# G1OJS/PyFT8

Hardware: AMD Instinct MI355X
Metric: FT8 15-s frames decoded/sec (higher is better)
Workload: dtype f32

## Files before the change

pyft8_amd/csrc/kernels/cycle_spectrum.hpp:

```cpp
#ifndef FT8RX_CYCLE_SPECTRUM_HPP
#define FT8RX_CYCLE_SPECTRUM_HPP

FT8_DEV void cyc_a_load(const int16_t* __restrict__ a, int n2b, int tid, uint32_t (&raw)[10]) {
#pragma unroll
    for (int q = 0; q < 10; q++) {
        const int i = tid + 256 * q, ic = i < 2400 ? i : 0;
        const int c = ic & 7, n1 = ic >> 3;
        const int m = 320 * n1 + n2b + c;
        const int inb = (2 * m < FT8RX_NSAMP) ? -1 : 0;
        raw[q] = *reinterpret_cast<const uint32_t*>(a + ((2 * m) & inb)) & (uint32_t)inb;
    }
}
FT8_DEV void cyc_a_frame(const uint32_t (&raw)[10], cpx* bufA, cpx* bufB, cpx* __restrict__ out, const Tables& T, int n2b, int tid) {
#pragma unroll
    for (int q = 0; q < 10; q++) {
        const int i = tid + 256 * q;
        if (i < 2400) bufA[(i & 7) * 300 + (i >> 3)] = make_float2((float)(int16_t)(raw[q] & 0xFFFFu), (float)(int16_t)(raw[q] >> 16));
    }
    cpx w[10];
#pragma unroll
    for (int q = 0; q < 10; q++) { const int i = tid + 256 * q, ic = i < 2400 ? i : 0; w[q] = T.W96000[(n2b + (ic & 7)) * (ic >> 3)]; }
    __syncthreads();
    cpx* r = lds_fft<300, 5, 5, 4, 3>(bufA, bufB, T.W300, 8, tid, 256);
#pragma unroll
    for (int q = 0; q < 10; q++) {
        const int i = tid + 256 * q;
        if (i < 2400) { const int c = i & 7, k1 = i >> 3; out[k1 * 320 + n2b + c] = cmul(r[c * 300 + k1], w[q]); }
    }
}
__global__ __launch_bounds__(256) void k_cyc_a(const int16_t* __restrict__ audio, cpx* __restrict__ A, Tables T) {
    __shared__ cpx bufA[8 * 300];
    __shared__ cpx bufB[8 * 300];
    static_assert(320 / 8 == 8 * 5, "the tile map below assumes 40 column tiles = 8 XCDs x 5");
    const int tile = (blockIdx.x & 7) * 5 + (blockIdx.x >> 3);
    const int f = blockIdx.y, tid = threadIdx.x, n2b = 8 * tile;
    uint32_t raw[10];
    cyc_a_load(audio + (size_t)f * FT8RX_NSAMP, n2b, tid, raw);
    cyc_a_frame(raw, bufA, bufB, A + (size_t)f * 96000, T, n2b, tid);
}

#define CYC_BC_BLOCKS 39
#define CYC_BC_GRID 40
FT8_DEV int cyc_bc_row(int b, int r) {
    if (b == CYC_BC_BLOCKS - 1) return (r == 0) ? 0 : 150;
    const int k1a = 1 + 4 * b;
    return (r < 4) ? k1a + r : 300 - (k1a + (r - 4));
}
FT8_DEV void cyc_bc_load(const cpx* __restrict__ in, int b, int tid, cpx (&v)[10]) {
#pragma unroll
    for (int q = 0; q < 10; q++) {
        const int i = tid + 256 * q, r = i / 320, c = i - 320 * r;
        v[q] = in[(size_t)cyc_bc_row(b, r) * 320 + c];
    }
}
FT8_DEV void cyc_bc_frame(const cpx (&v)[10], cpx* bufA, cpx* bufB, cpx* __restrict__ out, const Tables& T, int b, int tid) {
#pragma unroll
    for (int q = 0; q < 10; q++) bufA[tid + 256 * q] = v[q];
    __syncthreads();
    cpx* z = lds_fft<320, 8, 8, 5>(bufA, bufB, T.W320, 8, tid, 256);
    const bool special = (b == CYC_BC_BLOCKS - 1);
    constexpr int NK2 = (FT8RX_SPEC_BINS + 299) / 300;
    static_assert(NK2 <= 320, "k2 range of the 320-point row transforms");
    for (int i = tid; i < 8 * NK2; i += 256) {
        const int half = i / (4 * NK2), j = i - half * (4 * NK2), rr = j & 3, k2 = j >> 2;
        const int r = 4 * half + rr;
        int pr, pk2;
        if (special) {
            if (r >= 2) continue;
            pr = r;
            pk2 = (r == 0) ? ((320 - k2) % 320) : 319 - k2;
        } else {
            pr = (r < 4) ? r + 4 : r - 4;
            pk2 = 319 - k2;
        }
        const int k = cyc_bc_row(b, r) + 300 * k2;
        if (k >= FT8RX_SPEC_BINS) continue;
        const cpx p = z[r * 320 + k2], q = z[pr * 320 + pk2];
        const float er = 0.5f * (p.x + q.x), ei = 0.5f * (p.y - q.y);
        const float orr = 0.5f * (p.y + q.y), oi = 0.5f * (q.x - p.x);
        const cpx w = T.WR192k[k];
        out[k] = make_float2(er + (w.x * orr - w.y * oi), ei + (w.x * oi + w.y * orr));
    }
}
__global__ __launch_bounds__(256) void k_cyc_bc(const cpx* __restrict__ A, cpx* __restrict__ spec, Tables T) {
    __shared__ cpx bufA[8 * 320];
    __shared__ cpx bufB[8 * 320];
    static_assert(CYC_BC_GRID == 8 * 5 && CYC_BC_BLOCKS <= CYC_BC_GRID, "tile map: 40 slots = 8 XCDs x 5");
    const int f = blockIdx.y, tid = threadIdx.x, b = (blockIdx.x & 7) * 5 + (blockIdx.x >> 3);
    if (b >= CYC_BC_BLOCKS) return;
    cpx v[10];
    cyc_bc_load(A + (size_t)f * 96000, b, tid, v);
    cyc_bc_frame(v, bufA, bufB, spec + (size_t)f * FT8RX_SPEC_BINS, T, b, tid);
}

#endif
```

pyft8_amd/csrc/kernels/fine_sync.hpp:

```cpp
#ifndef FT8RX_FINE_SYNC_HPP
#define FT8RX_FINE_SYNC_HPP

#ifndef FINE_NT
#define FINE_NT 128
#endif
#ifndef FINE_WV
#define FINE_WV 3
#endif
#define FINE_INV 0.0003125f

#ifdef FINE_TIMING
__device__ unsigned long long g_fine_t[32];
#define FT_DECL __shared__ unsigned long long ft_l[32]; if (tid < 32) ft_l[tid] = 0; __syncthreads(); unsigned long long ft_prev = __builtin_readcyclecounter();
#define FT_ARG , unsigned long long& ft_prev, unsigned long long* ft_l
#define FT_PASS , ft_prev, ft_l
#define FT(i) do { if (tid == 0) { unsigned long long ft_now = __builtin_readcyclecounter(); ft_l[i] += ft_now - ft_prev; ft_prev = __builtin_readcyclecounter(); } } while (0)
#define FT_FLUSH do { __syncthreads(); if (tid < 32) atomicAdd(&g_fine_t[tid], ft_l[tid]); } while (0)
#else
#define FT_DECL
#define FT_ARG
#define FT_PASS
#define FT(i) do { } while (0)
#define FT_FLUSH do { } while (0)
#endif
// ... 2 lines not shown
FT8_DEV cpx fine_taper(cpx v, double t) { return make_float2((float)((double)v.x * t), (float)((double)v.y * t)); }
FT8_DEV cpx fine_conj(cpx v) { return make_float2(v.x, -v.y); }

FT8_DEV void dft8_in012(cpx* a) {
    const float h = 0.70710678f;
    const cpx a0 = a[0], a1 = a[1], a2 = a[2];
    const cpx e0 = cadd(a0, a2), e2 = csub(a0, a2);
    const cpx e1 = make_float2(a0.x + a2.y, a0.y - a2.x), e3 = make_float2(a0.x - a2.y, a0.y + a2.x);
    const cpx o1 = make_float2(h * (a1.x + a1.y), h * (a1.y - a1.x));
    const cpx o2 = make_float2(a1.y, -a1.x);
    const cpx o3 = make_float2(o1.y, -o1.x);
    a[0] = cadd(e0, a1); a[4] = csub(e0, a1);
    a[1] = cadd(e1, o1); a[5] = csub(e1, o1);
    a[2] = cadd(e2, o2); a[6] = csub(e2, o2);
    a[3] = cadd(e3, o3); a[7] = csub(e3, o3);
}
FT8_DEV void dft8_in017(cpx* a) {
    const float h = 0.70710678f;
    const cpx a0 = a[0], a1 = a[1], a7 = a[7];
    const cpx q0 = cadd(a1, a7), q2 = csub(a1, a7);
    const cpx q1 = make_float2(a1.x - a7.y, a1.y + a7.x), q3 = make_float2(a1.x + a7.y, a1.y - a7.x);
    const cpx o1 = make_float2(h * (q1.x + q1.y), h * (q1.y - q1.x));
    const cpx o2 = make_float2(q2.y, -q2.x);
    const cpx o3 = make_float2(h * (q3.y - q3.x), -(h * (q3.x + q3.y)));
    a[0] = cadd(a0, q0); a[4] = csub(a0, q0);
    a[1] = cadd(a0, o1); a[5] = csub(a0, o1);
    a[2] = cadd(a0, o2); a[6] = csub(a0, o2);
    a[3] = cadd(a0, o3); a[7] = csub(a0, o3);
}
static_assert(FINE_NT == 128, "fine_stage1 is written for 128 threads");
FT8_DEV void fine_stage1(const cpx* S, int fb, cpx* z, const cpx* __restrict__ W,
                         const double* __restrict__ taper, int tid FT_ARG) {
    const cpx zero = make_float2(0.0f, 0.0f);
    const cpx* s0 = S + fb + tid;
    const cpx* s7 = S + fb - 150 - 250 + tid;
    const cpx a00 = s0[0], a01 = s0[400];
    const cpx a10 = s0[128], a11 = s0[528];
    const cpx a20 = s0[256], a21 = s0[656];
    const bool r3 = tid < 16;
    const int t3 = r3 ? tid : 0;
    const cpx a30 = s0[384 + t3 - tid], a31 = s0[784 + t3 - tid];
    const bool has02 = tid < 50;
    const cpx a02r = s0[has02 ? 800 : 0];
    const double t02 = taper[has02 ? tid + 50 : 0];
    const bool has17 = tid >= 122;
    const cpx a17r = s7[has17 ? 128 : 250];
    const double t17 = taper[has17 ? tid - 122 : 0];
    const uint32_t m02 = has02 ? 0xFFFFFFFFu : 0u, m17 = has17 ? 0xFFFFFFFFu : 0u;
    const cpx a27r = s7[256];
    const bool tap21 = tid >= 94;
    const double t2 = taper[tap21 ? tid - 94 : tid + 6];
    const cpx a37r = s7[384 + t3 - tid];
    const double t31 = taper[34 + t3];
    const cpx t02v = fine_taper(a02r, t02), t17v = fine_taper(a17r, t17);
    const cpx a02 = make_float2(__uint_as_float(__float_as_uint(t02v.x) & m02), __uint_as_float(__float_as_uint(t02v.y) & m02));
    const cpx a17 = make_float2(__uint_as_float(__float_as_uint(t17v.x) & m17), __uint_as_float(__float_as_uint(t17v.y) & m17));
    const cpx sel2 = fine_taper(tap21 ? a21 : a27r, t2);
    const cpx b21 = tap21 ? sel2 : a21, a27 = tap21 ? a27r : sel2;
    const cpx b31 = fine_taper(a31, t31);
    cpx a[4][8];
#pragma unroll
    for (int i = 0; i < 4; i++)
#pragma unroll
        for (int j = 2; j < 7; j++) a[i][j] = zero;
    a[0][0] = fine_conj(a00); a[0][1] = fine_conj(a01); a[0][2] = fine_conj(a02); a[0][7] = zero;
    a[1][0] = fine_conj(a10); a[1][1] = fine_conj(a11); a[1][7] = fine_conj(a17);
    a[2][0] = fine_conj(a20); a[2][1] = fine_conj(b21); a[2][7] = fine_conj(a27);
    a[3][0] = fine_conj(a30); a[3][1] = fine_conj(b31); a[3][7] = fine_conj(a37r);
#pragma unroll
    for (int i = 0; i < 4; i++) {
        const int p = tid + 128 * i;
        const int pw = (i < 3) ? p : 384 + t3;
        cpx w[8];
#pragma unroll
        for (int j = 1; j < 8; j++) w[j] = W[j * pw];
        if (i == 0) dft8_in012(a[i]); else dft8_in017(a[i]);
#pragma unroll
        for (int j = 1; j < 8; j++) a[i][j] = cmul(a[i][j], w[j]);
        if (i < 3 || r3) {
#pragma unroll
            for (int j = 0; j < 8; j++) z[8 * p + j] = a[i][j];
        }
    }
    FT(1);
    __syncthreads();
    FT(2);
}
FT8_DEV void fine_stage2(cpx* z, const cpx* w400, int tid FT_ARG) {
    typedef Fused2<3200, 400, 8, 4, 4> F;
    constexpr int R = (F::groups + FINE_NT - 1) / FINE_NT;
    cpx a[R][4][4];
#pragma unroll
    for (int r = 0; r < R; r++) { const int g = tid + FINE_NT * r; if (g < F::groups) F::load_affine<200, 800>(z, g, a[r]); }
    FT(3);
    __syncthreads();
    FT(4);
#pragma unroll
    for (int r = 0; r < R; r++) {
        const int g = tid + FINE_NT * r;
        if (g < F::groups) {
            const int pp = g >> 3;
#pragma unroll
            for (int jp = 0; jp < 4; jp++) {
                dft<4>(a[r][jp]);
                const int pq = pp + 25 * jp;
#pragma unroll
                for (int j = 1; j < 4; j++) a[r][jp][j] = cmul(a[r][jp][j], w400[j * pq]);
            }
#pragma unroll
            for (int j = 0; j < 4; j++) {
                cpx b[4];
#pragma unroll
                for (int jp = 0; jp < 4; jp++) b[jp] = a[r][jp][j];
                dft<4>(b);
#pragma unroll
                for (int jp = 1; jp < 4; jp++) b[jp] = cmul(b[jp], w400[4 * jp * pp]);
#pragma unroll
                for (int jp = 0; jp < 4; jp++) a[r][jp][j] = b[jp];
            }
            F::store_affine<32, 8>(z, (g & 7) + 128 * (g >> 3), a[r]);
        }
    }
    FT(5);
    __syncthreads();
    FT(6);
}
FT8_DEV void fine_stage3(cpx* z, const cpx* __restrict__ W, int tid, int lo, int hi FT_ARG) {
    typedef Fused2<3200, 25, 128, 5, 5> F;
    constexpr int R = F::groups / FINE_NT;
    cpx a[R][5][5];
#pragma unroll
    for (int r = 0; r < R; r++) F::load_affine<128, 640>(z, tid + FINE_NT * r, a[r]);
    FT(7);
    __syncthreads();
    FT(8);
#pragma unroll
    for (int r = 0; r < R; r++) {
        const int q = tid + FINE_NT * r;
        F::compute_passA(0, a[r], W);
#pragma unroll
        for (int j = 0; j < 5; j++) {
            const int rr = q + 128 * j;
            const int first = rr + 640 * (lo / 640 + (rr < lo % 640 ? 1 : 0));
            if (first < hi && first < 3200) {
                cpx b[5];
#pragma unroll
                for (int jp = 0; jp < 5; jp++) b[jp] = a[r][jp][j];
                dft<5>(b);
#pragma unroll
                for (int jp = 0; jp < 5; jp++) z[rr + 640 * jp] = b[jp];
            }
        }
    }
    FT(9);
    __syncthreads();
    FT(10);
}
FT8_DEV void fine_fft(const cpx* S, int fb, cpx* z, const cpx* w400, const Tables& T, int tid, int lo, int hi FT_ARG) {
    FT(0);
    fine_stage1(S, fb, z, T.W3200, T.taper, tid FT_PASS);
    fine_stage2(z, w400, tid FT_PASS);
    fine_stage3(z, T.W3200, tid, lo, hi FT_PASS);
}

template <int NT>
FT8_DEV void fine_sym_quad(const cpx* z, int i0, int n2, const cpx* wq, float* mag) {
    if (i0 < 0) i0 = 0;
    if (i0 > 3168) i0 = 3168;
    cpx x[8];
#pragma unroll
    for (int n1 = 0; n1 < 8; n1++) { cpx v = z[i0 + 4 * n1 + n2]; x[n1] = make_float2(v.x * FINE_INV, -(v.y * FINE_INV)); }
    sym32_quad<NT>(x, n2, wq, mag);
}

#ifdef FT8RX_ILP_UNIT
#define FS_CS 0
#define FS_H 156
#define FS_MAG 1556
struct FsLane {
    float k[17];
    cpx g0[10];
    cpx g[10];
    double tap;
    cpx cs[2];
    int r, jlo;
};
FT8_DEV void fscore_fetch(FsLane& L, const Tables& T, int tid) {
    const int lane = tid & 63;
    const int ln = lane < 50 ? lane : 0;
    L.r = tid < 64 ? 50 + ln : ln;
    L.jlo = tid < 64 ? -2 : -1;
#pragma unroll
    for (int u = 0; u < 17; u++) L.k[u] = T.K32[900 + L.r + 100 * (L.jlo - 7 + u)];
#pragma unroll
    for (int q = 0; q < 10; q++) L.g0[q] = T.G1000[L.r + 100 * (L.jlo + q) + 150];
    L.tap = T.taper[tid < 64 ? ln : 50 + ln];
#pragma unroll
    for (int u = 0; u < 2; u++) { const int i = tid + FINE_NT * u; L.cs[u] = T.CS100[i < 156 ? i : 0]; }
}
FT8_DEV void fscore_phases(FsLane& L, const Tables& T, int nb0) {
    cpx w[10];
    {
        const int step = (((100 * nb0) % 3200) + 3200) % 3200;
        int idx = ((((L.r + 100 * L.jlo) * nb0) % 3200) + 3200) % 3200;
#pragma unroll
        for (int q = 0; q < 10; q++) { w[q] = T.W3200[idx]; idx += step; idx -= (idx >= 3200) ? 3200 : 0; }
    }
#pragma unroll
    for (int q = 0; q < 10; q++) L.g[q] = cmul(make_float2(w[q].x, -w[q].y), L.g0[q]);
}
FT8_DEV void fscore_prepare(FsLane& L, cpx* zi, const Tables& T, int nb0, int tid) {
    fscore_phases(L, T, nb0);
#pragma unroll
    for (int u = 0; u < 2; u++) { const int i = tid + FINE_NT * u; if (i < 156) zi[FS_CS + i] = L.cs[u]; }
    __syncthreads();
}
template <int NTONE>
FT8_DEV void fscore_p1(const cpx* S, int off, const FsLane& L, cpx* H, int tid FT_ARG) {
    cpx b[10];
#pragma unroll
    for (int q = 0; q < 10; q++) {
        cpx x = S[off + L.r + 100 * (L.jlo + q)];
        if (q == 0 || q == 9) x = fine_taper(x, L.tap);
        b[q] = cmul(x, L.g[q]);
    }
    FT(16);
    float hx[NTONE], hy[NTONE];
#pragma unroll
    for (int t = 0; t < NTONE; t++) { hx[t] = 0.0f; hy[t] = 0.0f; }
#pragma unroll
    for (int u = 0; u < 17; u++) {
#pragma unroll
        for (int t = 0; t < NTONE; t++) {
            const int q = u + t - 7;
            if (q >= 0 && q < 10) {
                hx[t] = __builtin_fmaf(b[q].x, L.k[u], hx[t]);
                hy[t] = __builtin_fmaf(b[q].y, L.k[u], hy[t]);
            }
        }
    }
    FT(17);
#pragma unroll
    for (int t = 0; t < NTONE; t++) H[t * 100 + L.r] = make_float2(hx[t], hy[t]);
}
FT8_DEV void dft10_fwd(const cpx* x, cpx* y) {
    cpx a0[5], a1[5];
#pragma unroll
    for (int n = 0; n < 5; n++) { const cpx u = x[(2 * n) % 10], v = x[(5 + 2 * n) % 10]; a0[n] = cadd(u, v); a1[n] = csub(u, v); }
    dft<5>(a0); dft<5>(a1);
#pragma unroll
    for (int k = 0; k < 5; k++) { y[(6 * k) % 10] = a0[k]; y[(5 + 6 * k) % 10] = a1[k]; }
}
FT8_DEV float row16_sum(float v) {
    v += __int_as_float(__builtin_amdgcn_update_dpp(0, __float_as_int(v), 0xB1, 0xf, 0xf, false));
    v += __int_as_float(__builtin_amdgcn_update_dpp(0, __float_as_int(v), 0x4E, 0xf, 0xf, false));
    v += __int_as_float(__builtin_amdgcn_update_dpp(0, __float_as_int(v), 0x141, 0xf, 0xf, false));
    v += __int_as_float(__builtin_amdgcn_update_dpp(0, __float_as_int(v), 0x140, 0xf, 0xf, false));
    return v;
}
FT8_DEV void fine_fscore(const cpx* S, int off, const FsLane& L, cpx* zi, int n, int tid FT_ARG) {
    cpx* H = zi + FS_H + (n & 1) * 700;
    float* mags = reinterpret_cast<float*>(zi + FS_MAG) + n * 56;
    const int lane = tid & 63;
    if (lane < 50) fscore_p1<7>(S, off, L, H, tid FT_PASS);
    FT(11);
    __syncthreads();
    FT(12);
    {
        const int c = tid & 15, t = tid >> 4;
        cpx acc[7];
#pragma unroll
        for (int s = 0; s < 7; s++) acc[s] = make_float2(0.0f, 0.0f);
        const cpx* Ht = H + (t < 7 ? t : 0) * 100;
#pragma unroll
        for (int i = 0; i < 2; i++) {
            const int p = c + 16 * i;
            if (i < 1 || c < 10) {
                const bool first = (i == 0 && c == 0), last = (i == 1 && c == 9);
                const cpx zero = make_float2(0.0f, 0.0f);
                const cpx h1 = Ht[p];
                cpx h2 = Ht[first ? 99 : 100 - p], h3 = Ht[50 - p], h4 = Ht[50 + p];
                if (first) { h2 = zero; h4 = zero; }
                if (last) { h3 = zero; h4 = zero; }
                const cpx P = make_float2(h1.x + h2.x, h1.y + h2.y), M = make_float2(h1.x - h2.x, h1.y - h2.y);
                const cpx P2 = make_float2(h3.x + h4.x, h3.y + h4.y), M2 = make_float2(h3.x - h4.x, h3.y - h4.y);
                const cpx A = make_float2(P.x + P2.x, P.y + P2.y), B = make_float2(P.x - P2.x, P.y - P2.y);
                const cpx C = make_float2(M.x - M2.x, M.y - M2.y), D = make_float2(M.x + M2.x, M.y + M2.y);
                acc[0] = cadd(acc[0], A);
#pragma unroll
                for (int s = 1; s < 7; s++) {
                    const cpx e = zi[FS_CS + (s - 1) * 26 + p];
                    const cpx X = (s & 1) ? B : A, Y = (s & 1) ? D : C;
                    acc[s].x = __builtin_fmaf(X.x, e.x, __builtin_fmaf(-Y.y, e.y, acc[s].x));
                    acc[s].y = __builtin_fmaf(X.y, e.x, __builtin_fmaf(Y.x, e.y, acc[s].y));
                }
            }
        }
        FT(19);
#pragma unroll
        for (int s = 0; s < 7; s++) { acc[s].x = row16_sum(acc[s].x); acc[s].y = row16_sum(acc[s].y); }
        {
            cpx v = acc[0];
#pragma unroll
            for (int s = 1; s < 7; s++) v = (c == s) ? acc[s] : v;
            const float re = v.x * FINE_INV, im = v.y * FINE_INV;
            mags[c < 7 ? c * 8 + t : 7] = sqrtf(re * re + im * im);
        }
    }
    FT(14);
}

FT8_DEV void fine_candidate(int tid, int bid, const cpx* __restrict__ spec, ft8rx_record* __restrict__ rec,
                            const int32_t* __restrict__ ncand, float* __restrict__ llr0, const Tables& T, const ft8rx_config& cfg,
                            const int32_t* __restrict__ trip, int32_t* __restrict__ t_out ,
                            float* __restrict__ t_sd, float* __restrict__ t_sgrid) {
    __shared__ cpx z[3200];
    __shared__ cpx w400[400];
    float* mg = reinterpret_cast<float*>(w400);
    static_assert(sizeof(cpx) * 400 >= sizeof(float) * 640, "mg overlays w400");
    __shared__ cpx w32[32];
    __shared__ float sc[16];
    __shared__ int ish[4];
    const int lane = tid & 63;
    int frame, ci = 0, f0, h0;
    if (trip) { frame = trip[3 * bid]; f0 = trip[3 * bid + 1]; h0 = trip[3 * bid + 2]; }
    else {
        frame = bid >> cand_shift(cfg); ci = bid & ((1 << cand_shift(cfg)) - 1);
        if (ci >= ncand[frame]) return;
        const ft8rx_record& r = rec[bid];
        if (r.status != FT8RX_ST_ACTIVE) return;
        f0 = r.f0_idx; h0 = r.h0_idx;
    }
    if (h0 < FT8RX_MIN_H0_FD || h0 > FT8RX_MAX_H0_FD) return;
    const cpx w32v = T.W32[tid & 31];
    const int fb0 = 50 * f0;
    {
        constexpr int NW = (400 + FINE_NT - 1) / FINE_NT;
        cpx wv[NW];
#pragma unroll
        for (int q = 0; q < NW; q++) { const int i = tid + FINE_NT * q; wv[q] = T.W3200[8 * (i < 400 ? i : 0)]; }
#pragma unroll
        for (int q = 0; q < NW; q++) { const int i = tid + FINE_NT * q; if (i < 400) w400[i] = wv[q]; }
        if (tid < 32) w32[tid] = w32v;
        __syncthreads();
    }
    const cpx* __restrict__ Sg = spec + (size_t)frame * FT8RX_SPEC_BINS + (fb0 - 182);
    FT_DECL
    cpx wq[8];
    sym32_twiddles(w32, tid & 3, wq);
    const int tb0 = 8 * h0 + (h0 < 0 ? 1 : 0);
    double* dsum = reinterpret_cast<double*>(mg);
    fine_fft(Sg, 182, z, w400, T, tid, tb0 - 8 + 32 * 36, tb0 + 6 + 32 * 43 FT_PASS);
    FsLane L;
    fscore_fetch(L, T, tid);
    const bool lowslice = tb0 >= 667;
    cpx* slice = z + (lowslice ? 0 : 2048);
    cpx* zi = z + (lowslice ? 1152 : 0);
    static_assert(9 * 128 <= 1152 && 2048 + 9 * 128 <= 3200 && 1152 + 1780 <= 3200 && 1780 <= 2048, "slice copy and scan tables share the image");
    {
        const int wv = tid >> 6, ln = tid & 63;
#pragma unroll
        for (int c = 0; c < 5; c++) {
            const int ch = wv + 2 * c;
            if (ch < 9)
                __builtin_amdgcn_global_load_lds((const __attribute__((address_space(1))) void*)(Sg + 128 * ch + 2 * ln),
                                                 (__attribute__((address_space(3))) void*)(slice + 128 * ch), 16, 0, 0);
        }
    }
    const cpx* S = slice;
    float* p = reinterpret_cast<float*>(slice);
    float* llr = p + 464;
    float* sq = llr + 176;
#pragma unroll 1
    for (int r = 0; r < (224 + FINE_NT - 1) / FINE_NT; r++) {
        const int task = tid + FINE_NT * r, qd = task >> 2, n2 = task & 3;
        const bool valid = qd < 56;
        const int ti = valid ? qd / 7 : 0, a = valid ? qd - 7 * ti : 0;
        float mag[8];
        fine_sym_quad<7>(z, tb0 - 8 + 2 * ti + 32 * (36 + a), n2, wq, mag);
#pragma unroll
        for (int b = 0; b < 7; b++) asm volatile("" :: "v"(mag[b]));
        if (valid && n2 == 0) {
            const int c = d_COSTAS[a];
            double off = 0.0, on = 0.0;
#pragma unroll
            for (int b = 0; b < 7; b++) { const double m = (double)mag[b]; on = (b == c) ? m : on; off += (b == c) ? 0.0 : m; }
            dsum[(ti * 7 + a) * 2] = on; dsum[(ti * 7 + a) * 2 + 1] = off;
        }
    }
    FT(25);
    __syncthreads();
    int tt = -8; float score_f0 = 0.0f;
    {
        const int ti = tid & 7;
        double s1 = 0.0, s2 = 0.0;
#pragma unroll
        for (int a = 0; a < 7; a++) { s1 += dsum[(ti * 7 + a) * 2]; s2 += dsum[(ti * 7 + a) * 2 + 1]; }
        const float sct = (float)(s1 + W6 * s2);
#pragma unroll
        for (int u = 0; u < 8; u++) {
            const float v = __int_as_float(__builtin_amdgcn_readlane(__float_as_int(sct), u));
            if (u == 0 || v > score_f0) { score_f0 = v; tt = -8 + 2 * u; }
        }
    }
    FT(26);
    float best = 0.0f; int ft = 0;
    __builtin_amdgcn_s_waitcnt(0x0F70);
    fscore_prepare(L, zi, T, tb0 + tt + 32 * 36, tid);
    FT(18);
#pragma unroll 1
    for (int n = 0; n < 8; n++) {
        fine_fscore(S, 182 - 32 + 8 * (n < 4 ? n : n + 1), L, zi, n, tid FT_PASS);
        FT(15);
    }
    __syncthreads();
    if (tid < 56) {
        const int n = tid / 7, a = tid - 7 * n, c = d_COSTAS[a];
        const float* mags = reinterpret_cast<const float*>(zi + FS_MAG) + n * 56 + a * 8;
        double off = 0.0, on = 0.0;
#pragma unroll
        for (int b = 0; b < 7; b++) { const double m = (double)mags[b]; on = (b == c) ? m : on; off += (b == c) ? 0.0 : m; }
        dsum[tid * 2] = on; dsum[tid * 2 + 1] = off;
    }
    __syncthreads();
    {
        const int n = tid & 7;
        double s1 = 0.0, s2 = 0.0;
#pragma unroll
        for (int a = 0; a < 7; a++) { s1 += dsum[(n * 7 + a) * 2]; s2 += dsum[(n * 7 + a) * 2 + 1]; }
        const float sct = (float)(s1 + W6 * s2);
#pragma unroll
        for (int i = 0; i < 9; i++) {
            const float v = (i == 4) ? score_f0 : __int_as_float(__builtin_amdgcn_readlane(__float_as_int(sct), i < 4 ? i : i - 1));
            if (i == 0 || v > best) { best = v; ft = -32 + 8 * i; }
        }
    }
    FT(20);
    const int tb = tb0 + tt;
    cpx* Hc = zi;
    cpx* Ab = zi + 800;
    {
        const int t = (tid < 80) ? tid / 10 : 0, c10 = (tid < 80) ? tid - 10 * t : 0;
        cpx tw[9];
#pragma unroll
        for (int s1 = 1; s1 < 10; s1++) tw[s1 - 1] = T.TW100[c10 * s1];
        fscore_phases(L, T, tb);
        if (lane < 50) fscore_p1<8>(S, 182 + ft, L, Hc, tid FT_PASS);
        __syncthreads();
        FT(21);
        if (tid < 80) {
            cpx x[10], y[10];
#pragma unroll
            for (int r1 = 0; r1 < 10; r1++) { const cpx h = Hc[t * 100 + 10 * r1 + c10]; x[r1] = make_float2(h.x, -h.y); }
            dft10_fwd(x, y);
            Ab[t * 100 + c10] = y[0];
#pragma unroll
            for (int s1 = 1; s1 < 10; s1++) Ab[t * 100 + 10 * s1 + c10] = cmul(y[s1], tw[s1 - 1]);
        }
        __syncthreads();
        FT(22);
        if (tid < 80) {
            cpx x[10], y[10];
#pragma unroll
            for (int r2 = 0; r2 < 10; r2++) x[r2] = Ab[t * 100 + 10 * c10 + r2];
            dft10_fwd(x, y);
#pragma unroll
            for (int s2 = 0; s2 < 8; s2++) {
                const int sy = c10 + 10 * s2;
                const float re = y[s2].x * FINE_INV, im = y[s2].y * FINE_INV;
                if (sy < 79) mg[sy * 8 + t] = sqrtf(re * re + im * im);
            }
        }
    }
    const int n_lo = (tb < 0) ? min(79, (-tb) / 32 + 1) : 0;
    const int s_strict = (tb > 3168) ? 0 : (3168 - tb) / 32 + 1;
    const int s_up = (s_strict < 79) ? max(0, (3168 - tb + 31) / 32) : 79;
    if (n_lo > 0 || s_up < 79) {
        __syncthreads();
        fscore_phases(L, T, n_lo > 0 ? 0 : 3168);
        if (lane < 50) fscore_p1<8>(S, 182 + ft, L, Hc, tid FT_PASS);
        __syncthreads();
        const int c = tid & 15, t = tid >> 4;
        float ax = 0.0f, ay = 0.0f;
#pragma unroll
        for (int i = 0; i < 7; i++) {
            if (i < 6 || c < 4) { const cpx h = Hc[t * 100 + c + 16 * i]; ax = ax + h.x; ay = ay + h.y; }
        }
        ax = row16_sum(ax); ay = row16_sum(ay);
        const float re = ax * FINE_INV, im = ay * FINE_INV;
        const float m = sqrtf(re * re + im * im);
        if (n_lo > 0) { for (int sy = c; sy < n_lo; sy += 16) mg[sy * 8 + t] = m; }
        else { for (int sy = s_up + c; sy < 79; sy += 16) mg[sy * 8 + t] = m; }
    }
    __syncthreads();
    FT(23);
    bool match = false;
    if (tid < 21) {
        int blk = tid / 7, a = tid - blk * 7;
        const float* q = mg + 8 * (36 * blk + a);
        int am = 0; for (int t = 1; t < 8; t++) if (q[t] > q[am]) am = t;
        match = (am == d_COSTAS[a]);
    }
    if (tid < 64) { int nm = __popcll(__ballot(match)); if (tid == 0) ish[1] = nm; }
    __syncthreads();
    const int nsync = ish[1];
    FT(24);
    if (trip && t_sgrid) for (int i = tid; i < 632; i += FINE_NT) t_sgrid[(size_t)bid * 632 + i] = mg[i];
    int ret = 1; float sd = 0.0f; int snr = 0;
    if (nsync <= 6) ret = 0;
    else {
        for (int i = tid; i < 464; i += FINE_NT) p[i] = 20.0f * ft8_log10f(mg[8 * (int)d_PAYSYM[i >> 3] + (i & 7)]);
        __syncthreads();
// ... 268 lines not shown
```

pyft8_amd/csrc/kernels/subtract.hpp:

```cpp
#ifndef FT8RX_SUBTRACT_HPP
#define FT8RX_SUBTRACT_HPP

#define SUB_L (79 * 1920)
#define SUB_NCH 128
#define SUB_CH (SUB_L / SUB_NCH)

struct SubTables { const double* pulse; const double* pc; };

FT8_DEV void sub_signal(const ft8rx_subsig& S, const double* __restrict__ cum , const SubTables& T, int m, float* sr, float* si) {
    const int n = m + 1920;
    const double dphi_peak = 6.283185307179586 / 1920.0;
    int ih = n / 1920; if (ih > 78) ih = 78;
    const int il = ih - 2 > 0 ? ih - 2 : 0;
    double acc = cum[il] * T.pc[5759];
    for (int i = il; i <= ih; i++) {
        int j = n - 1920 * i; if (j > 5759) j = 5759;
        acc += (double)S.tones[i] * T.pc[j];
    }
    double phi = dphi_peak * acc + 6.283185307179586 * (S.fHz - 0.5) * (double)n / 12000.0;
    if (n < 3840) phi += dphi_peak * T.pulse[1920 + n] * (double)S.tones[0];
    if (n >= 79 * 1920) phi += dphi_peak * T.pulse[n - 79 * 1920] * (double)S.tones[78];
    const double rev = phi * (1.0 / 6.283185307179586);
    const float fr = (float)(rev - floor(rev));
    const float s = __builtin_amdgcn_sinf(fr), c = __builtin_amdgcn_cosf(fr);
// ... 291 lines not shown
        const int zi = 2 * q + zh;
        if (zi < sh.n) scan[((size_t)frame * SUB_MAXSHIFT + zi) * SUB_NCH + c] = make_double2((double)ar[q], (double)ai[q]);
    }
}

__global__ __launch_bounds__(256) void k_subd_accum(const float2* __restrict__ zdec, const float2* __restrict__ model,
                                                    const ft8rx_subsig* __restrict__ sigs, const int32_t* __restrict__ counts, int max_sigs,
                                                    int s, const SubdCtx* __restrict__ ctx, float2* __restrict__ adec ) {
    __shared__ double pr[4][20], pi_[4][20];
    __shared__ float Ar[20], Ai[20];
    const int frame = blockIdx.x, tid = threadIdx.x, wave = tid >> 6, lane = tid & 63;
    if (s >= counts[frame]) return;
    const ft8rx_subsig& S = sigs[(size_t)frame * max_sigs + s];
    const int s0 = (int)(12000.0 * S.tsec);
    const bool ok = s0 > 0 && s0 + SUB_L <= FT8RX_NSAMP;
    const int off = (s0 - ctx[frame].s00) / SUBD_D;
    const float2* z = zdec + (size_t)frame * SUBD_NZ + SUBD_PAD + off;
    const float2* w = model + (size_t)frame * SUBD_N;
    float fr_[20], fi_[20];
#pragma unroll
    for (int k = 0; k < 20; k++) { fr_[k] = 0.0f; fi_[k] = 0.0f; }
    for (int m = tid; m < SUBD_N; m += 256) {
        const float2 zv = z[m], wv = w[m];
        const float yr = zv.x * wv.x - zv.y * wv.y, yi = zv.x * wv.y + zv.y * wv.x;
        const float rv = (float)(SUBD_D * m) * (1.0f / 192000.0f);
        const float wr = __builtin_amdgcn_cosf(rv), wi = -__builtin_amdgcn_sinf(rv);
        float rr = 1.0f, ri = 0.0f;
#pragma unroll
        for (int k = 0; k < 20; k++) {
            fr_[k] += yr * rr - yi * ri; fi_[k] += yr * ri + yi * rr;
            const float t = rr * wr - ri * wi; ri = rr * wi + ri * wr; rr = t;
        }
    }
#pragma unroll
    for (int k = 0; k < 20; k++) {
        double vr = (double)fr_[k], vi = (double)fi_[k];
        for (int o = 32; o > 0; o >>= 1) { vr += __shfl_xor(vr, o); vi += __shfl_xor(vi, o); }
        if (lane == 0) { pr[wave][k] = vr; pi_[wave][k] = vi; }
    }
    __syncthreads();
    if (tid < 20) {
        const double sc = ok ? (double)SUBD_D / 192000.0 : 0.0;
        Ar[tid] = (float)(((pr[0][tid] + pr[1][tid]) + (pr[2][tid] + pr[3][tid])) * sc);
        Ai[tid] = (float)(((pi_[0][tid] + pi_[1][tid]) + (pi_[2][tid] + pi_[3][tid])) * sc);
    }
    __syncthreads();
    for (int m = tid; m <= SUBD_N; m += 256) {
        const float rv = (float)(SUBD_D * m) * (1.0f / 192000.0f);
        const float wr = __builtin_amdgcn_cosf(rv), wi = __builtin_amdgcn_sinf(rv);
        float rr = 1.0f, ri = 0.0f, er = 0.0f, ei = 0.0f;
#pragma unroll
        for (int k = 0; k < 20; k++) {
            er += Ar[k] * rr - Ai[k] * ri; ei += Ar[k] * ri + Ai[k] * rr;
            const float t = rr * wr - ri * wi; ri = rr * wi + ri * wr; rr = t;
        }
        adec[(size_t)frame * (SUBD_N + 1) + m] = make_float2(er, ei);
    }
}

__global__ __launch_bounds__(256) void k_subd_apply(float* __restrict__ wf, const ft8rx_subsig* __restrict__ sigs,
                                                    const int32_t* __restrict__ counts, int max_sigs, int s, SubTables T,
                                                    const float2* __restrict__ adec) {
    __shared__ ft8rx_subsig S;
    __shared__ double cum[80];
    const int frame = blockIdx.y, tid = threadIdx.x, wave = tid >> 6, lane = tid & 63;
    int s0;
    if (!sub_setup(sigs, counts, max_sigs, s, frame, &S, cum, &s0)) return;
    float* x = wf + (size_t)frame * FT8RX_NSAMP + s0;
    const float2* a = adec + (size_t)frame * (SUBD_N + 1);
    for (int i = 0; i < SUB_CPW; i++) {
        const int ch = (blockIdx.x * 4 + wave) * SUB_CPW + i;
        for (int m = ch * SUB_CH + lane; m < (ch + 1) * SUB_CH; m += 64) {
            float sr, si;
            sub_signal(S, cum, T, m, &sr, &si);
            int md = m >> 5; if (md > SUBD_N - 1) md = SUBD_N - 1;
            const float2 a0 = a[md], a1 = a[md + 1];
            float fq = (float)(m - SUBD_D * md) * (1.0f / 32.0f); if (fq > 1.0f) fq = 1.0f;
            const float er = a0.x + fq * (a1.x - a0.x), ei = a0.y + fq * (a1.y - a0.y);
            x[m] = x[m] - 2.0f * (er * sr - ei * si);
        }
    }
}

FT8_DEV void cyc_a_load_f32(const float* __restrict__ a, int n2b, int tid, float2 (&raw)[10]) {
#pragma unroll
    for (int q = 0; q < 10; q++) {
        const int i = tid + 256 * q, ic = i < 2400 ? i : 0;
        const int c = ic & 7, n1 = ic >> 3;
        const int m = 320 * n1 + n2b + c;
        const int inb = (2 * m < FT8RX_NSAMP) ? -1 : 0;
        const float2 v = *reinterpret_cast<const float2*>(a + ((2 * m) & inb));
        raw[q] = make_float2(__uint_as_float(__float_as_uint(v.x) & (uint32_t)inb), __uint_as_float(__float_as_uint(v.y) & (uint32_t)inb));
    }
}
__global__ __launch_bounds__(256) void k_cyc_a_f32(const float* __restrict__ audio, cpx* __restrict__ A, Tables T) {
    __shared__ cpx bufA[8 * 300];
    __shared__ cpx bufB[8 * 300];
    const int tile = (blockIdx.x & 7) * 5 + (blockIdx.x >> 3);
    const int f = blockIdx.y, tid = threadIdx.x, n2b = 8 * tile;
    float2 raw[10];
    cyc_a_load_f32(audio + (size_t)f * FT8RX_NSAMP, n2b, tid, raw);
#pragma unroll
    for (int q = 0; q < 10; q++) { const int i = tid + 256 * q; if (i < 2400) bufA[(i & 7) * 300 + (i >> 3)] = raw[q]; }
    cpx w[10];
#pragma unroll
    for (int q = 0; q < 10; q++) { const int i = tid + 256 * q, ic = i < 2400 ? i : 0; w[q] = T.W96000[(n2b + (ic & 7)) * (ic >> 3)]; }
    __syncthreads();
    cpx* r = lds_fft<300, 5, 5, 4, 3>(bufA, bufB, T.W300, 8, tid, 256);
    cpx* out = A + (size_t)f * 96000;
#pragma unroll
    for (int q = 0; q < 10; q++) {
        const int i = tid + 256 * q;
        if (i < 2400) { const int c = i & 7, k1 = i >> 3; out[k1 * 320 + n2b + c] = cmul(r[c * 300 + k1], w[q]); }
    }
}

__global__ __launch_bounds__(FINE_NT) void k_refine3(const cpx* __restrict__ spec, ft8rx_subsig* __restrict__ sigs, const int32_t* __restrict__ counts,
                                                     int max_sigs, int s, Tables T) {
    __shared__ cpx z[3200];
    __shared__ cpx slice[FINE_SLICE];
    __shared__ cpx w400[400];
    __shared__ cpx w32[32];
    __shared__ __attribute__((aligned(8))) double dsum[12 * 21 * 2];
    const int frame = blockIdx.x, tid = threadIdx.x;
    if (s >= counts[frame]) return;
    ft8rx_subsig& S = sigs[(size_t)frame * max_sigs + s];
    const int fb0 = (int)(0.5 + S.fHz * 16.0);
    const int tb0 = (int)(0.5 + S.tsec * 200.0);
    if (fb0 - 182 < 0 || fb0 - 182 + FINE_SLICE > FT8RX_SPEC_BINS) return;
    const cpx* Sg = spec + (size_t)frame * FT8RX_SPEC_BINS + (fb0 - 182);
    for (int i = tid; i < FINE_SLICE; i += FINE_NT) slice[i] = Sg[i];
    for (int i = tid; i < 400; i += FINE_NT) w400[i] = T.W3200[8 * i];
    if (tid < 32) w32[tid] = T.W32[tid];
    __syncthreads();
    cpx wq[8];
    sym32_twiddles(w32, tid & 3, wq);
    FT_DECL
    fine_fft(slice, 182, z, w400, T, tid, 0, 3200 FT_PASS);
#pragma unroll 1
    for (int r = 0; r < (12 * 21 * 4 + FINE_NT - 1) / FINE_NT; r++) {
        const int task = tid + FINE_NT * r, qd = task >> 2, n2 = task & 3;
        const bool valid = qd < 12 * 21;
        const int ti = valid ? qd / 21 : 0, sy = valid ? qd - 21 * ti : 0;
        const int blk = sy / 7, a = sy - 7 * blk;
        float mag[8];
        fine_sym_quad<7>(z, tb0 - 6 + ti + 32 * (36 * blk + a), n2, wq, mag);
        if (valid && n2 == 0) { double on, off; fine_onoff(mag, a, on, off); dsum[(ti * 21 + sy) * 2] = on; dsum[(ti * 21 + sy) * 2 + 1] = off; }
    }
    __syncthreads();
    if (tid == 0) {
        float best = 0.0f; int tbest = tb0 - 6;
        for (int ti = 0; ti < 12; ti++) {
            float sc = 0.0f;
            for (int blk = 0; blk < 3; blk++) {
                double s1 = 0.0, s2 = 0.0;
                for (int a = 0; a < 7; a++) { s1 += dsum[(ti * 21 + 7 * blk + a) * 2]; s2 += dsum[(ti * 21 + 7 * blk + a) * 2 + 1]; }
                const float sb = (float)(s1 + W6 * s2);
                if (blk == 0 || sb > sc) sc = sb;
            }
            if (ti == 0 || sc > best) { best = sc; tbest = tb0 - 6 + ti; }
        }
        S.tsec = (double)tbest / 200.0;
        S.fHz = (double)fb0 / 16.0;
    }
}

__global__ void k_sub_to_f32(const int16_t* __restrict__ a, float* __restrict__ wf, size_t n) {
    const size_t i = (size_t)blockIdx.x * blockDim.x + threadIdx.x;
    if (i < n) wf[i] = (float)a[i];
}
__global__ void k_sub_to_i16(const float* __restrict__ wf, int16_t* __restrict__ a, size_t n) {
    const size_t i = (size_t)blockIdx.x * blockDim.x + threadIdx.x;
    if (i < n) { float v = rintf(wf[i]); v = v > 32767.0f ? 32767.0f : (v < -32768.0f ? -32768.0f : v); a[i] = (int16_t)v; }
}

#endif
```

Measured before the change: 88810.

## Run cycle-A FFT in place in one LDS buffer; drop k_fine twiddle table

The cycle-spectrum column kernel replaces the generic two-buffer 300-point LDS FFT with a hand-scheduled in-place 5x5x12 decomposition. The first radix-5 pass runs straight from the global loads in registers, and the int16 and f32 variants share one templated tile routine. LDS use per block halves and launch bounds request more waves per CU. In k_fine the 400-entry LDS twiddle table is removed: stage 2 reads strided twiddles from the global W3200 table, and the score scratch arrays are overlaid onto free regions of the FFT image, so more blocks fit per CU. The cost is extra barriers, more global twiddle reads, and fragile overlay aliasing guarded by static_asserts.

Result: faster. 92360 (median of 6 runs) (+4.0%).

```diff
diff --git a/pyft8_amd/csrc/kernels/cycle_spectrum.hpp b/pyft8_amd/csrc/kernels/cycle_spectrum.hpp
--- a/pyft8_amd/csrc/kernels/cycle_spectrum.hpp
+++ b/pyft8_amd/csrc/kernels/cycle_spectrum.hpp
@@ -1,42 +1,122 @@
 #ifndef FT8RX_CYCLE_SPECTRUM_HPP
 #define FT8RX_CYCLE_SPECTRUM_HPP
 
-FT8_DEV void cyc_a_load(const int16_t* __restrict__ a, int n2b, int tid, uint32_t (&raw)[10]) {
+template <class LD>
+FT8_DEV void cyc_a_tile(const LD& ld, cpx* X, cpx* __restrict__ out, const Tables& T, int n2b, int tid) {
+    const cpx* __restrict__ W = T.W300;
+    {
+        typename LD::raw_t raw[2][5];
 #pragma unroll
-    for (int q = 0; q < 10; q++) {
-        const int i = tid + 256 * q, ic = i < 2400 ? i : 0;
-        const int c = ic & 7, n1 = ic >> 3;
-        const int m = 320 * n1 + n2b + c;
-        const int inb = (2 * m < FT8RX_NSAMP) ? -1 : 0;
-        raw[q] = *reinterpret_cast<const uint32_t*>(a + ((2 * m) & inb)) & (uint32_t)inb;
+        for (int r = 0; r < 2; r++) {
+            const int b = tid + 256 * r, bc = b < 480 ? b : 0;
+            const int c = bc & 7, p = bc >> 3;
+#pragma unroll
+            for (int j = 0; j < 5; j++) raw[r][j] = ld.fetch(320 * (p + 60 * j) + n2b + c);
+        }
+#pragma unroll
+        for (int r = 0; r < 2; r++) {
+            const int b = tid + 256 * r, bc = b < 480 ? b : 0;
+            const int c = bc & 7, p = bc >> 3;
+            cpx a[5], w[5];
+#pragma unroll
+            for (int j = 1; j < 5; j++) w[j] = W[j * p];
+#pragma unroll
+            for (int j = 0; j < 5; j++) a[j] = ld.conv(raw[r][j]);
+            dft<5>(a);
+#pragma unroll
+            for (int j = 1; j < 5; j++) a[j] = cmul(a[j], w[j]);
+            if (b < 480) {
+#pragma unroll
+                for (int j = 0; j < 5; j++) X[c * 300 + 5 * p + j] = a[j];
+            }
+        }
     }
-}
-FT8_DEV void cyc_a_frame(const uint32_t (&raw)[10], cpx* bufA, cpx* bufB, cpx* __restrict__ out, const Tables& T, int n2b, int tid) {
+    __syncthreads();
+    cpx w4[10];
+    {
+        cpx a[2][5];
+#pragma unroll
+        for (int r = 0; r < 2; r++) {
+            const int b = tid + 256 * r, bc = b < 480 ? b : 0;
+            const int seq = bc / 60, bb = bc - 60 * seq;
+#pragma unroll
+            for (int j = 0; j < 5; j++) a[r][j] = X[seq * 300 + bb + 60 * j];
+        }
+        __syncthreads();
+#pragma unroll
+        for (int r = 0; r < 2; r++) {
+            const int b = tid + 256 * r, bc = b < 480 ? b : 0;
+            const int seq = bc / 60, bb = bc - 60 * seq, p = bb / 5, q = bb - 5 * p;
+            cpx w[5];
+#pragma unroll
+            for (int j = 1; j < 5; j++) w[j] = W[j * p * 5];
+            dft<5>(a[r]);
+#pragma unroll
+            for (int j = 1; j < 5; j++) a[r][j] = cmul(a[r][j], w[j]);
+            if (b < 480) {
+#pragma unroll
+                for (int j = 0; j < 5; j++) X[seq * 300 + q + 25 * p + 5 * j] = a[r][j];
+            }
+        }
+        __syncthreads();
+    }
+    {
+        typedef Fused2<300, 12, 25, 4, 3> F;
+        static_assert(F::groups == 25 && F::m2 == 1, "one twelve-point group per q; the last pass is twiddle-free");
+        const int g = tid < 200 ? tid : 0, seq = g / 25, q = g - 25 * seq;
+        cpx a[3][4];
+        F::load_affine<25, 75>(X, seq * 300 + q, a);
+        cpx w[3][4];
+#pragma unroll
+        for (int jp = 0; jp < 3; jp++)
+#pragma unroll
+            for (int j = 1; j < 4; j++) w[jp][j] = W[j * jp * 25];
+        __syncthreads();
+#pragma unroll
+        for (int jp = 0; jp < 3; jp++) {
+            dft<4>(a[jp]);
+#pragma unroll
+            for (int j = 1; j < 4; j++) a[jp][j] = cmul(a[jp][j], w[jp][j]);
+        }
+#pragma unroll
+        for (int j = 0; j < 4; j++) {
+            cpx b[3];
+#pragma unroll
+            for (int jp = 0; jp < 3; jp++) b[jp] = a[jp][j];
+            dft<3>(b);
+#pragma unroll
+            for (int jp = 0; jp < 3; jp++) a[jp][j] = b[jp];
+        }
+        if (tid < 200) F::store_affine<100, 25>(X, seq * 300 + q, a);
+        asm volatile("" ::: "memory");
+#pragma unroll
+        for (int q = 0; q < 10; q++) { const int i = tid + 256 * q, ic = i < 2400 ? i : 0; w4[q] = T.W96000[(n2b + (ic & 7)) * (ic >> 3)]; }
+        __syncthreads();
+    }
 #pragma unroll
     for (int q = 0; q < 10; q++) {
         const int i = tid + 256 * q;
-        if (i < 2400) bufA[(i & 7) * 300 + (i >> 3)] = make_float2((float)(int16_t)(raw[q] & 0xFFFFu), (float)(int16_t)(raw[q] >> 16));
-    }
-    cpx w[10];
-#pragma unroll
-    for (int q = 0; q < 10; q++) { const int i = tid + 256 * q, ic = i < 2400 ? i : 0; w[q] = T.W96000[(n2b + (ic & 7)) * (ic >> 3)]; }
-    __syncthreads();
-    cpx* r = lds_fft<300, 5, 5, 4, 3>(bufA, bufB, T.W300, 8, tid, 256);
-#pragma unroll
-    for (int q = 0; q < 10; q++) {
-        const int i = tid + 256 * q;
-        if (i < 2400) { const int c = i & 7, k1 = i >> 3; out[k1 * 320 + n2b + c] = cmul(r[c * 300 + k1], w[q]); }
+        if (i < 2400) { const int c = i & 7, k1 = i >> 3; out[k1 * 320 + n2b + c] = cmul(X[c * 300 + k1], w4[q]); }
     }
 }
-__global__ __launch_bounds__(256) void k_cyc_a(const int16_t* __restrict__ audio, cpx* __restrict__ A, Tables T) {
-    __shared__ cpx bufA[8 * 300];
-    __shared__ cpx bufB[8 * 300];
-    static_assert(320 / 8 == 8 * 5, "the tile map below assumes 40 column tiles = 8 XCDs x 5");
-    const int tile = (blockIdx.x & 7) * 5 + (blockIdx.x >> 3);
-    const int f = blockIdx.y, tid = threadIdx.x, n2b = 8 * tile;
-    uint32_t raw[10];
-    cyc_a_load(audio + (size_t)f * FT8RX_NSAMP, n2b, tid, raw);
-    cyc_a_frame(raw, bufA, bufB, A + (size_t)f * 96000, T, n2b, tid);
+static_assert(320 / 8 == 8 * 5, "the tile map below assumes 40 column tiles = 8 XCDs x 5");
+FT8_DEV int cyc_a_tile_of_block(int bx) { return (bx & 7) * 5 + (bx >> 3); }
+struct CycLoadI16 {
+    const int16_t* __restrict__ a;
+    typedef uint32_t raw_t;
+    FT8_DEV raw_t fetch(int m) const {
+        const int inb = (2 * m < FT8RX_NSAMP) ? -1 : 0;
+        return *reinterpret_cast<const uint32_t*>(a + ((2 * m) & inb)) & (uint32_t)inb;
+    }
+    FT8_DEV cpx conv(raw_t v) const { return make_float2((float)(int16_t)(v & 0xFFFFu), (float)(int16_t)(v >> 16)); }
+};
+#ifndef CYC_A_WV
+#define CYC_A_WV 8
+#endif
+__global__ __launch_bounds__(256, CYC_A_WV) void k_cyc_a(const int16_t* __restrict__ audio, cpx* __restrict__ A, Tables T) {
+    __shared__ cpx X[8 * 300];
+    const int f = blockIdx.y, n2b = 8 * cyc_a_tile_of_block(blockIdx.x);
+    cyc_a_tile(CycLoadI16{audio + (size_t)f * FT8RX_NSAMP}, X, A + (size_t)f * 96000, T, n2b, threadIdx.x);
 }
 
 #define CYC_BC_BLOCKS 39
diff --git a/pyft8_amd/csrc/kernels/fine_sync.hpp b/pyft8_amd/csrc/kernels/fine_sync.hpp
--- a/pyft8_amd/csrc/kernels/fine_sync.hpp
+++ b/pyft8_amd/csrc/kernels/fine_sync.hpp
@@ -108,13 +108,13 @@
             for (int j = 0; j < 8; j++) z[8 * p + j] = a[i][j];
         }
     }
-    FT(1);
-    __syncthreads();
-    FT(2);
-}
-FT8_DEV void fine_stage2(cpx* z, const cpx* w400, int tid FT_ARG) {
-    typedef Fused2<3200, 400, 8, 4, 4> F;
-    constexpr int R = (F::groups + FINE_NT - 1) / FINE_NT;
+}
+typedef Fused2<3200, 400, 8, 4, 4> FineF2;
+#define FINE_R2 ((FineF2::groups + FINE_NT - 1) / FINE_NT)
+template <int STRIDE>
+FT8_DEV void fine_stage2(cpx* z, const cpx* __restrict__ w, int tid FT_ARG) {
+    typedef FineF2 F;
+    constexpr int R = FINE_R2;
     cpx a[R][4][4];
 #pragma unroll
     for (int r = 0; r < R; r++) { const int g = tid + FINE_NT * r; if (g < F::groups) F::load_affine<200, 800>(z, g, a[r]); }
@@ -129,9 +129,8 @@
 #pragma unroll
             for (int jp = 0; jp < 4; jp++) {
                 dft<4>(a[r][jp]);
-                const int pq = pp + 25 * jp;
-#pragma unroll
-                for (int j = 1; j < 4; j++) a[r][jp][j] = cmul(a[r][jp][j], w400[j * pq]);
+#pragma unroll
+                for (int j = 1; j < 4; j++) a[r][jp][j] = cmul(a[r][jp][j], w[STRIDE * (j * (pp + 25 * jp))]);
             }
 #pragma unroll
             for (int j = 0; j < 4; j++) {
@@ -140,7 +139,7 @@
                 for (int jp = 0; jp < 4; jp++) b[jp] = a[r][jp][j];
                 dft<4>(b);
 #pragma unroll
-                for (int jp = 1; jp < 4; jp++) b[jp] = cmul(b[jp], w400[4 * jp * pp]);
+                for (int jp = 1; jp < 4; jp++) b[jp] = cmul(b[jp], w[STRIDE * (4 * jp * pp)]);
 #pragma unroll
                 for (int jp = 0; jp < 4; jp++) a[r][jp][j] = b[jp];
             }
@@ -182,10 +181,14 @@
     __syncthreads();
     FT(10);
 }
+template <bool LDSW = true>
 FT8_DEV void fine_fft(const cpx* S, int fb, cpx* z, const cpx* w400, const Tables& T, int tid, int lo, int hi FT_ARG) {
     FT(0);
     fine_stage1(S, fb, z, T.W3200, T.taper, tid FT_PASS);
-    fine_stage2(z, w400, tid FT_PASS);
+    FT(1);
+    __syncthreads();
+    FT(2);
+    if (LDSW) fine_stage2<1>(z, w400, tid FT_PASS); else fine_stage2<8>(z, T.W3200, tid FT_PASS);
     fine_stage3(z, T.W3200, tid, lo, hi FT_PASS);
 }
 
@@ -340,13 +343,14 @@
                             const int32_t* __restrict__ ncand, float* __restrict__ llr0, const Tables& T, const ft8rx_config& cfg,
                             const int32_t* __restrict__ trip, int32_t* __restrict__ t_out ,
                             float* __restrict__ t_sd, float* __restrict__ t_sgrid) {
-    __shared__ cpx z[3200];
-    __shared__ cpx w400[400];
-    float* mg = reinterpret_cast<float*>(w400);
-    static_assert(sizeof(cpx) * 400 >= sizeof(float) * 640, "mg overlays w400");
+#ifndef FINE_LDS_PAD
+#define FINE_LDS_PAD 0
+#endif
+    __shared__ cpx z[3200 + FINE_LDS_PAD];
     __shared__ cpx w32[32];
     __shared__ float sc[16];
     __shared__ int ish[4];
+    static_assert(sizeof(cpx) * (3200 + FINE_LDS_PAD + 32) + sizeof(float) * 16 + sizeof(int) * 4 <= (FINE_LDS_PAD ? 32768 : 26880), "k_fine: six blocks per CU need <= 21 granules of 1280 B");
     const int lane = tid & 63;
     int frame, ci = 0, f0, h0;
     if (trip) { frame = trip[3 * bid]; f0 = trip[3 * bid + 1]; h0 = trip[3 * bid + 2]; }
@@ -358,31 +362,26 @@
         f0 = r.f0_idx; h0 = r.h0_idx;
     }
     if (h0 < FT8RX_MIN_H0_FD || h0 > FT8RX_MAX_H0_FD) return;
-    const cpx w32v = T.W32[tid & 31];
     const int fb0 = 50 * f0;
-    {
-        constexpr int NW = (400 + FINE_NT - 1) / FINE_NT;
-        cpx wv[NW];
-#pragma unroll
-        for (int q = 0; q < NW; q++) { const int i = tid + FINE_NT * q; wv[q] = T.W3200[8 * (i < 400 ? i : 0)]; }
-#pragma unroll
-        for (int q = 0; q < NW; q++) { const int i = tid + FINE_NT * q; if (i < 400) w400[i] = wv[q]; }
-        if (tid < 32) w32[tid] = w32v;
-        __syncthreads();
-    }
+    if (tid < 32) w32[tid] = T.W32[tid];
     const cpx* __restrict__ Sg = spec + (size_t)frame * FT8RX_SPEC_BINS + (fb0 - 182);
     FT_DECL
+    const int tb0 = 8 * h0 + (h0 < 0 ? 1 : 0);
+    fine_fft<false>(Sg, 182, z, nullptr, T, tid, tb0 - 8 + 32 * 36, tb0 + 6 + 32 * 43 FT_PASS);
     cpx wq[8];
     sym32_twiddles(w32, tid & 3, wq);
-    const int tb0 = 8 * h0 + (h0 < 0 ? 1 : 0);
-    double* dsum = reinterpret_cast<double*>(mg);
-    fine_fft(Sg, 182, z, w400, T, tid, tb0 - 8 + 32 * 36, tb0 + 6 + 32 * 43 FT_PASS);
     FsLane L;
     fscore_fetch(L, T, tid);
     const bool lowslice = tb0 >= 667;
     cpx* slice = z + (lowslice ? 0 : 2048);
     cpx* zi = z + (lowslice ? 1152 : 0);
     static_assert(9 * 128 <= 1152 && 2048 + 9 * 128 <= 3200 && 1152 + 1780 <= 3200 && 1780 <= 2048, "slice copy and scan tables share the image");
+    static_assert(1152 + 156 + 112 <= 667 + 1144 && 156 + 112 <= 268 && 268 + 238 <= 1024 && 1024 + 112 <= 2048, "time-scan sums: clear of the scoring reads, the slice copy and the (cos, sin) table");
+    static_assert(1152 + 1780 + 112 <= 3200 && 1780 + 112 <= 2048, "frequency-scan sums: behind the scan tables, clear of the slice");
+    static_assert(1152 + 1600 + 316 <= 3200 && 1600 + 316 <= 2048 && 2 * 316 >= 79 * 8, "final grid: behind Hc + Ab, clear of the slice");
+    double* dsum = reinterpret_cast<double*>(z + (lowslice ? 1152 + 156 : (tb0 + 1144 >= 268 ? 156 : 1024)));
+    double* dsumf = reinterpret_cast<double*>(z + (lowslice ? 1152 + 1780 : 1780));
+    float* mg = reinterpret_cast<float*>(z + (lowslice ? 1152 + 1600 : 1600));
     {
         const int wv = tid >> 6, ln = tid & 63;
 #pragma unroll
@@ -446,14 +445,14 @@
         double off = 0.0, on = 0.0;
 #pragma unroll
         for (int b = 0; b < 7; b++) { const double m = (double)mags[b]; on = (b == c) ? m : on; off += (b == c) ? 0.0 : m; }
-        dsum[tid * 2] = on; dsum[tid * 2 + 1] = off;
+        dsumf[tid * 2] = on; dsumf[tid * 2 + 1] = off;
     }
     __syncthreads();
     {
         const int n = tid & 7;
         double s1 = 0.0, s2 = 0.0;
 #pragma unroll
-        for (int a = 0; a < 7; a++) { s1 += dsum[(n * 7 + a) * 2]; s2 += dsum[(n * 7 + a) * 2 + 1]; }
+        for (int a = 0; a < 7; a++) { s1 += dsumf[(n * 7 + a) * 2]; s2 += dsumf[(n * 7 + a) * 2 + 1]; }
         const float sct = (float)(s1 + W6 * s2);
 #pragma unroll
         for (int i = 0; i < 9; i++) {
diff --git a/pyft8_amd/csrc/kernels/subtract.hpp b/pyft8_amd/csrc/kernels/subtract.hpp
--- a/pyft8_amd/csrc/kernels/subtract.hpp
+++ b/pyft8_amd/csrc/kernels/subtract.hpp
@@ -397,37 +397,20 @@
     }
 }
 
-FT8_DEV void cyc_a_load_f32(const float* __restrict__ a, int n2b, int tid, float2 (&raw)[10]) {
-#pragma unroll
-    for (int q = 0; q < 10; q++) {
-        const int i = tid + 256 * q, ic = i < 2400 ? i : 0;
-        const int c = ic & 7, n1 = ic >> 3;
-        const int m = 320 * n1 + n2b + c;
+struct CycLoadF32 {
+    const float* __restrict__ a;
+    typedef float2 raw_t;
+    FT8_DEV raw_t fetch(int m) const {
         const int inb = (2 * m < FT8RX_NSAMP) ? -1 : 0;
         const float2 v = *reinterpret_cast<const float2*>(a + ((2 * m) & inb));
-        raw[q] = make_float2(__uint_as_float(__float_as_uint(v.x) & (uint32_t)inb), __uint_as_float(__float_as_uint(v.y) & (uint32_t)inb));
-    }
-}
-__global__ __launch_bounds__(256) void k_cyc_a_f32(const float* __restrict__ audio, cpx* __restrict__ A, Tables T) {
-    __shared__ cpx bufA[8 * 300];
-    __shared__ cpx bufB[8 * 300];
-    const int tile = (blockIdx.x & 7) * 5 + (blockIdx.x >> 3);
-    const int f = blockIdx.y, tid = threadIdx.x, n2b = 8 * tile;
-    float2 raw[10];
-    cyc_a_load_f32(audio + (size_t)f * FT8RX_NSAMP, n2b, tid, raw);
-#pragma unroll
-    for (int q = 0; q < 10; q++) { const int i = tid + 256 * q; if (i < 2400) bufA[(i & 7) * 300 + (i >> 3)] = raw[q]; }
-    cpx w[10];
-#pragma unroll
-    for (int q = 0; q < 10; q++) { const int i = tid + 256 * q, ic = i < 2400 ? i : 0; w[q] = T.W96000[(n2b + (ic & 7)) * (ic >> 3)]; }
-    __syncthreads();
-    cpx* r = lds_fft<300, 5, 5, 4, 3>(bufA, bufB, T.W300, 8, tid, 256);
-    cpx* out = A + (size_t)f * 96000;
-#pragma unroll
-    for (int q = 0; q < 10; q++) {
-        const int i = tid + 256 * q;
-        if (i < 2400) { const int c = i & 7, k1 = i >> 3; out[k1 * 320 + n2b + c] = cmul(r[c * 300 + k1], w[q]); }
-    }
+        return make_float2(__uint_as_float(__float_as_uint(v.x) & (uint32_t)inb), __uint_as_float(__float_as_uint(v.y) & (uint32_t)inb));
+    }
+    FT8_DEV cpx conv(raw_t v) const { return v; }
+};
+__global__ __launch_bounds__(256, CYC_A_WV) void k_cyc_a_f32(const float* __restrict__ audio, cpx* __restrict__ A, Tables T) {
+    __shared__ cpx X[8 * 300];
+    const int f = blockIdx.y, n2b = 8 * cyc_a_tile_of_block(blockIdx.x);
+    cyc_a_tile(CycLoadF32{audio + (size_t)f * FT8RX_NSAMP}, X, A + (size_t)f * 96000, T, n2b, threadIdx.x);
 }
 
 __global__ __launch_bounds__(FINE_NT) void k_refine3(const cpx* __restrict__ spec, ft8rx_subsig* __restrict__ sigs, const int32_t* __restrict__ counts,
```
